# turboderp-org/exllamav2

Hardware: NVIDIA H100
Metric: decode tokens/sec (bs=1) Llama2-7B EXL2-4.0bpw (higher is better)
Workload: dtype fp16 (int2-8 weights, fp32 accumulate)

## Files before the change

exllamav2_b200/csrc/common.cuh:

```cuda
#pragma once
#include <cuda_fp16.h>
#include <cuda_runtime.h>
#include <stdint.h>
#include <stdio.h>
#include <stdlib.h>
#include <string.h>

#include <atomic>

#include "../../include/exl2_b200.h"
#include "layout.h"

namespace exl2b {

void set_error(const char* fmt, ...);
extern std::atomic<uint64_t> g_launch_count;

#define EXL2B_CUDA(call)                                                                              \
    do {                                                                                              \
        cudaError_t _e = (call);                                                                      \
        if (_e != cudaSuccess) {                                                                      \
            exl2b::set_error("%s failed: %s (%s:%d)", #call, cudaGetErrorString(_e), __FILE__, __LINE__); \
            return -1;                                                                                \
        }                                                                                             \
// ... 83 lines not shown
        : "memory");
}
__device__ __forceinline__ void bulk_copy_g2s(uint32_t dst_smem, const void* src, uint32_t bytes, uint32_t bar) {
    asm volatile("cp.async.bulk.shared::cluster.global.mbarrier::complete_tx::bytes [%0], [%1], %2, [%3];" ::"r"(dst_smem),
                 "l"(src), "r"(bytes), "r"(bar)
                 : "memory");
}

__device__ __forceinline__ void bulk_prefetch_l2(const void* src, uint32_t bytes) {
    asm volatile("cp.async.bulk.prefetch.L2.global [%0], %1;" ::"l"(src), "r"(bytes) : "memory");
}

__device__ __forceinline__ void mma16816(float (&d)[4], const uint32_t* a, uint32_t b0, uint32_t b1) {
    asm("mma.sync.aligned.m16n8k16.row.col.f32.f16.f16.f32 {%0,%1,%2,%3}, {%4,%5,%6,%7}, {%8,%9}, {%0,%1,%2,%3};"
        : "+f"(d[0]), "+f"(d[1]), "+f"(d[2]), "+f"(d[3])
        : "r"(a[0]), "r"(a[1]), "r"(a[2]), "r"(a[3]), "r"(b0), "r"(b1));
}

__device__ __forceinline__ uint4 lds128(uint32_t addr) {
    uint4 v;
    asm volatile("ld.shared.v4.u32 {%0,%1,%2,%3}, [%4];" : "=r"(v.x), "=r"(v.y), "=r"(v.z), "=r"(v.w) : "r"(addr));
    return v;
}
__device__ __forceinline__ uint2 lds64(uint32_t addr) {
    uint2 v;
    asm volatile("ld.shared.v2.u32 {%0,%1}, [%2];" : "=r"(v.x), "=r"(v.y) : "r"(addr));
    return v;
}
__device__ __forceinline__ uint32_t lds32(uint32_t addr) {
    uint32_t v;
    asm volatile("ld.shared.u32 %0, [%1];" : "=r"(v) : "r"(addr));
    return v;
}
#endif

}
```

exllamav2_b200/csrc/gemv_i8.cu:

```cuda
#include <string.h>

#include <algorithm>
#include <map>
#include <mutex>
#include <string>
#include <vector>

#include "gemv_i8.cuh"

namespace exl2b {

constexpr int I8_MAX_WARPS = 16;
constexpr int I8_MAX_CTAS = 320;

struct I8Mat {
    const uint8_t* packed;
    const void* wtab;
    const half* bias;
    half* c;
    half* c_perm;
    const uint16_t* out_invperm;
    int N, blk_base, clear;
};

constexpr uint32_t DF_FLUSH = 1, DF_BLOCK_DONE = 2, DF_GPTQ = 4;
constexpr int I8_BARS = 8;

struct I8Params {
    I8Mat mat[I8_MAX_MATS];
    const uint4* plan_desc;
    const uint32_t* plan_first;
    const uint32_t* plan_cta;
    const uint32_t* plan_red;
    int num_mats, K, KS;
    const uint16_t* perm;
    const half* x;
    const half* x2;
    const half* norm_w;
    float norm_eps;
    int mode, x_permuted;
    int norm_permuted;
    int l1_hints;
    int l2_prefetch;
    int arena;
    int busy_ctas;
    unsigned int* slot_cnt;
    unsigned long long* dbg;
    int dbg_cta;
    unsigned long long* dbg_rec;
};

struct I8Smem {
    uint32_t act, asum, ascale, emit, total;
};
__host__ __device__ inline I8Smem i8_smem_map(int warps, int arena, int KS) {
    auto up = [](uint32_t x) { return (x + 15u) & ~15u; };
    I8Smem m;
    m.act = up((uint32_t)warps * (uint32_t)arena);
    m.asum = up(m.act + (uint32_t)KS * 64u);
    m.ascale = up(m.asum + (uint32_t)KS * 4u);
    m.emit = up(m.ascale + (uint32_t)(KS / 4 + 1) * 4u);
    m.total = up(m.emit + (uint32_t)warps * 256u);
    return m;
}

__device__ __forceinline__ int dp4a_us(uint32_t a, uint32_t b, int c) {
    int d;
    asm("dp4a.u32.s32 %0, %1, %2, %3;" : "=r"(d) : "r"(a), "r"(b), "r"(c));
    return d;
}
__device__ __forceinline__ int dp4a_uu(uint32_t a, uint32_t b, int c) {
    int d;
    asm("dp4a.u32.u32 %0, %1, %2, %3;" : "=r"(d) : "r"(a), "r"(b), "r"(c));
    return d;
}

__device__ __forceinline__ uint4 ldg_keep(const uint4* p) {
    uint4 v;
    asm volatile("ld.global.nc.L1::evict_last.v4.u32 {%0,%1,%2,%3}, [%4];" : "=r"(v.x), "=r"(v.y), "=r"(v.z), "=r"(v.w) : "l"(p));
    return v;
}
__device__ __forceinline__ uint32_t ldg_pass_u16(const void* p) {
    unsigned short v;
    asm volatile("ld.global.nc.L1::no_allocate.u16 %0, [%1];" : "=h"(v) : "l"(p));
    return v;
}
__device__ __forceinline__ uint32_t ldg_pass_u32(const void* p) {
    uint32_t v;
    asm volatile("ld.global.nc.L1::no_allocate.u32 %0, [%1];" : "=r"(v) : "l"(p));
    return v;
}

template <int BITS>
__device__ __forceinline__ void consume_slab(uint32_t wb, uint32_t xs, int lane, int (&am)[4], int (&ae)[2]) {
    constexpr int Pm = plane_main(BITS), Pe = plane_extra(BITS);
    if constexpr (BITS == 4) {
        const uint4 w4 = lds128(wb + lane * 16);
#pragma unroll
        for (int hf = 0; hf < 2; ++hf) {
            const uint4 xh = lds128(xs + hf * 16), xl = lds128(xs + 32 + hf * 16);
            const uint32_t wa = hf ? w4.z : w4.x, wc = hf ? w4.w : w4.y;
            const uint32_t lo0 = wa & 0x0f0f0f0fu, hi0 = wa & 0xf0f0f0f0u, lo1 = wc & 0x0f0f0f0fu, hi1 = wc & 0xf0f0f0f0u;
            am[0] = dp4a_us(lo0, xh.x, am[0]);
            am[1] = dp4a_uu(lo0, xl.x, am[1]);
            am[2] = dp4a_us(hi0, xh.y, am[2]);
            am[3] = dp4a_uu(hi0, xl.y, am[3]);
            am[0] = dp4a_us(lo1, xh.z, am[0]);
            am[1] = dp4a_uu(lo1, xl.z, am[1]);
            am[2] = dp4a_us(hi1, xh.w, am[2]);
            am[3] = dp4a_uu(hi1, xl.w, am[3]);
        }
        return;
    }
    uint32_t XH[8], XL[8];
    {
        const uint4 h0 = lds128(xs), h1 = lds128(xs + 16), l0 = lds128(xs + 32), l1 = lds128(xs + 48);
        XH[0] = h0.x; XH[1] = h0.y; XH[2] = h0.z; XH[3] = h0.w; XH[4] = h1.x; XH[5] = h1.y; XH[6] = h1.z; XH[7] = h1.w;
        XL[0] = l0.x; XL[1] = l0.y; XL[2] = l0.z; XL[3] = l0.w; XL[4] = l1.x; XL[5] = l1.y; XL[6] = l1.z; XL[7] = l1.w;
    }
    if constexpr (Pm == 4) {
        const uint4 w4 = lds128(wb + lane * 16);
        const uint32_t W[4] = {w4.x, w4.y, w4.z, w4.w};
#pragma unroll
// ... 144 lines not shown
#define I8_STAMP(i) do { if (P.dbg) { if (blockIdx.x == P.dbg_cta && tid == 0) P.dbg[i] = i8_gtimer(); if ((i) == 0 && tid == 0) atomicMin(P.dbg + 6, i8_gtimer()); } } while (0)

template <int I8_WARPS>
__global__ void __launch_bounds__(I8_WARPS * 32, 2) gemv_i8_kernel(const __grid_constant__ I8Params P) {
    constexpr int I8_THREADS = I8_WARPS * 32;
    extern __shared__ __align__(128) uint8_t smem[];
    __shared__ uint64_t bars[I8_WARPS * I8_BARS];
    __shared__ float s_red[I8_WARPS];

    const int tid = threadIdx.x, warp = tid >> 5, lane = tid & 31;
    const int KS = P.KS;
    I8_STAMP(0);
    if (P.dbg_rec && tid == 0 && blockIdx.x < 160) P.dbg_rec[blockIdx.x * 4] = i8_gtimer();
    if (tid < I8_WARPS * I8_BARS) mbar_init(smem_addr(&bars[tid]), 1);
    mbar_fence_init();
    __syncthreads();
    griddep_launch_dependents();

    if ((int)blockIdx.x >= P.busy_ctas) {
        if (tid == 0) {
            while (*reinterpret_cast<volatile unsigned int*>(P.slot_cnt) < (unsigned)P.busy_ctas) __nanosleep(200);
            if (atomicAdd(P.slot_cnt, 1u) == gridDim.x - 1u) *reinterpret_cast<volatile unsigned int*>(P.slot_cnt) = 0u;
        }
        return;
    }

    const uint32_t cinfo = __ldg(P.plan_cta + blockIdx.x);
    const int blk0 = (int)(cinfo & 0xffffu), nb = (int)(cinfo >> 16);
    const uint32_t fw0 = __ldg(P.plan_first + blockIdx.x * I8_WARPS + warp), fw1 = __ldg(P.plan_first + blockIdx.x * I8_WARPS + warp + 1);
    const uint32_t f0 = fw0 & 0x3ffffffu, f1 = fw1 & 0x3ffffffu;
    const int nst = (int)(f1 - f0), n_pre = (int)(fw0 >> 26);
    const uint4* const list = P.plan_desc + f0;

    const I8Smem sm = i8_smem_map(I8_WARPS, P.arena, KS);
    uint8_t* const act_g = smem + sm.act;
    int* const asum_s = reinterpret_cast<int*>(smem + sm.asum);
    float* const ascale_s = reinterpret_cast<float*>(smem + sm.ascale);
    float* const emit_base = reinterpret_cast<float*>(smem + sm.emit);
    uint32_t sbase;
    asm volatile("mov.u32 %0, %1;" : "=r"(sbase) : "r"(smem_addr(smem)));
    const uint32_t ring = sbase + (uint32_t)warp * (uint32_t)P.arena;
    const uint32_t act = sbase + sm.act, asum = sbase + sm.asum, ascale = sbase + sm.ascale;
    uint32_t bar0;
    asm volatile("mov.u32 %0, %1;" : "=r"(bar0) : "r"(smem_addr(&bars[warp * I8_BARS])));

    uint32_t mi_cur = 0u;
    const uint8_t* pk_cur = P.mat[0].packed;
    const uint8_t* wt_cur = reinterpret_cast<const uint8_t*>(P.mat[0].wtab);
    auto select_mat = [&](uint32_t mi) {
        if (mi != mi_cur) {
            mi_cur = mi;
            pk_cur = mi == 0 ? P.mat[0].packed : (mi == 1 ? P.mat[1].packed : P.mat[2].packed);
            wt_cur = reinterpret_cast<const uint8_t*>(mi == 0 ? P.mat[0].wtab : (mi == 1 ? P.mat[1].wtab : P.mat[2].wtab));
        }
    };
    auto issue_stages = [&](int s0, int cnt, uint4 d) {
        if (lane < cnt) {
            const int s = s0 + lane;
            const uint32_t mi = (d.z >> 22) & 3u;
            const uint8_t* pk = mi == 0 ? P.mat[0].packed : (mi == 1 ? P.mat[1].packed : P.mat[2].packed);
            const uint32_t bytes = ((d.z >> 24) & 0xffu) << 7;
            const uint32_t bar = bar0 + ((uint32_t)s & (I8_BARS - 1)) * 8u;
            mbar_arrive_expect_tx(bar, bytes);
            bulk_copy_g2s(ring + ((d.w >> 16) & 0xffu) * 128u, pk + d.x, bytes, bar);
        }
    };
    auto load_req = [&](int s0) -> uint4 {
        uint4 d = make_uint4(0u, 0u, 0u, 0u);
        if (lane < I8_BARS && s0 + lane < nst) d = P.l1_hints ? ldg_keep(list + s0 + lane) : __ldg(list + s0 + lane);
        return d;
    };
    auto fetch_scale = [&](uint4 d) -> uint32_t {
        select_mat((d.z >> 22) & 3u);
        const uint32_t idx = d.y + (uint32_t)lane;
        if (P.l1_hints)
            return (d.z & (DF_GPTQ << 18)) ? ldg_pass_u32(reinterpret_cast<const uint32_t*>(wt_cur) + idx)
                                            : ldg_pass_u16(reinterpret_cast<const unsigned short*>(wt_cur) + idx);
        return (d.z & (DF_GPTQ << 18)) ? __ldg(reinterpret_cast<const uint32_t*>(wt_cur) + idx)
                                        : (uint32_t)__ldg(reinterpret_cast<const unsigned short*>(wt_cur) + idx);
    };
    uint4 dcur = make_uint4(0u, 0u, 0u, 0u);
    if (nst > 0) dcur = P.l1_hints ? ldg_keep(list) : __ldg(list);
    I8_STAMP(8);
    issue_stages(0, n_pre, load_req(0));
    int next_req = n_pre;
    if (P.l2_prefetch)
        for (int s0 = n_pre; s0 < nst; s0 += 32) {
            const int s = s0 + lane;
            if (s < nst) {
                const uint4 d = __ldg(list + s);
                const uint32_t mi = (d.z >> 22) & 3u;
                const uint8_t* pk = mi == 0 ? P.mat[0].packed : (mi == 1 ? P.mat[1].packed : P.mat[2].packed);
                bulk_prefetch_l2(pk + d.x, ((d.z >> 24) & 0xffu) << 7);
            }
        }
    uint32_t wraw = 0u;
    if (nst > 0) wraw = fetch_scale(dcur);
    I8_STAMP(9);

    const int n_oct = P.K >> 3;
    const bool gather_x = P.perm != nullptr && !P.x_permuted;
    constexpr int PF = 3;
    uint4 pv[PF], wv[PF];
#pragma unroll
    for (int r = 0; r < PF; ++r) {
        const int o = r * I8_THREADS + tid;
        pv[r] = make_uint4(0, 0, 0, 0);
        wv[r] = make_uint4(0, 0, 0, 0);
        if (o < n_oct) {
            if (P.perm && (gather_x || !P.norm_permuted)) pv[r] = __ldg(reinterpret_cast<const uint4*>(P.perm + o * 8));
            if (P.mode == I8_RMSNORM) {
                if (P.perm && !P.norm_permuted) {
                    const uint16_t* pi = reinterpret_cast<const uint16_t*>(&pv[r]);
                    uint16_t* wo = reinterpret_cast<uint16_t*>(&wv[r]);
#pragma unroll
                    for (int e = 0; e < 8; ++e) wo[e] = __half_as_ushort(__ldg(P.norm_w + pi[e]));
                } else {
                    wv[r] = __ldg(reinterpret_cast<const uint4*>(P.norm_w + o * 8));
                }
            }
        }
    }

    I8_STAMP(1);
    griddep_wait();
    I8_STAMP(2);
    if (P.dbg_rec && tid == 0 && blockIdx.x < 160) P.dbg_rec[blockIdx.x * 4 + 1] = i8_gtimer();

    float sumsq = 0.f;
    const bool two_in = (P.mode == I8_SILU_MUL || P.mode == I8_GELU_MUL);
// ... 110 lines not shown
                    wreg = __ldg(reinterpret_cast<const uint4*>(P.norm_w + o * 8));
                }
            }
        }
        stage_round(o, pidx, wreg, false, make_uint4(0, 0, 0, 0));
    }
    if (P.mode == I8_RMSNORM) {
#pragma unroll
        for (int s = 16; s > 0; s >>= 1) sumsq += __shfl_xor_sync(0xffffffffu, sumsq, s);
        if (lane == 0) s_red[warp] = sumsq;
    }
    __syncthreads();
    I8_STAMP(3);
    float rrms = 1.f;
    if (P.mode == I8_RMSNORM) {
        float t = 0.f;
#pragma unroll
        for (int i = 0; i < I8_WARPS; ++i) t += s_red[i];
        rrms = rsqrtf(t * (1.0f / (float)P.K) + P.norm_eps);
    }

    uint32_t red0 = 0u;
    I8OutPre opre0 = {0u, 0u};
    if (warp < nb) {
        red0 = __ldg(P.plan_red + blk0 + warp);
        if (red0 & 0xffffu) opre0 = out_pre(P, blk0 + warp, lane);
    }

    int am[4] = {0, 0, 0, 0}, ae[2] = {0, 0};
    float tot = 0.f;
    int S = 0, blk_slabs = 0, emits = 0;
#pragma unroll 1
    for (int s = 0; s < nst; ++s) {
        const uint4 d = dcur;
        if (s + 1 < nst) dcur = P.l1_hints ? ldg_keep(list + s + 1) : __ldg(list + s + 1);
        const int nreq = (int)((d.w >> 24) & 15u);
        const uint4 dreq = load_req(next_req);
        mbar_wait(bar0 + ((uint32_t)s & (I8_BARS - 1)) * 8u, ((uint32_t)s >> 3) & 1u);
        const int ks = (int)(d.z & 0x7ffu), n = (int)((d.z >> 11) & 7u), bits = (int)((d.z >> 14) & 15u);
        const uint32_t slot = ring + ((d.w >> 16) & 0xffu) * 128u;
        const uint32_t xs = act + (uint32_t)ks * 64u, as = asum + (uint32_t)ks * 4u;
        {
            int bsel = bits;
            auto opaque = [&]() { asm volatile("" : "+r"(bsel)); return bsel; };
            if (bsel == 4) S += consume_stage<4>(slot, n, xs, as, lane, am, ae);
            else if (opaque() == 5) S += consume_stage<5>(slot, n, xs, as, lane, am, ae);
            else if (opaque() == 6) S += consume_stage<6>(slot, n, xs, as, lane, am, ae);
            else if (opaque() == 3) S += consume_stage<3>(slot, n, xs, as, lane, am, ae);
            else if (opaque() == 8) S += consume_stage<8>(slot, n, xs, as, lane, am, ae);
            else S += consume_stage<2>(slot, n, xs, as, lane, am, ae);
        }
        __syncwarp();
        {
            issue_stages(next_req, nreq, dreq);
            next_req += nreq;
        }
        blk_slabs += n;
        if (d.z & (DF_FLUSH << 18)) {
            int v = ((am[0] << 8) + am[1]) + (((am[2] << 8) + am[3]) >> 4) + (((ae[0] << 8) + ae[1]) << plane_main(bits));
            const float ws = __half2float(__ushort_as_half((unsigned short)(wraw & 0xffffu)));
            const int zero = (d.z & (DF_GPTQ << 18)) ? (int)(wraw >> 16) : (1 << (bits - 1));
            v -= zero * S;
            tot = fmaf((float)v, ws * __uint_as_float(lds32(ascale + (uint32_t)(ks >> 2) * 4u)), tot);
            am[0] = am[1] = am[2] = am[3] = 0;
            ae[0] = ae[1] = 0;
            S = 0;
            if (s + 1 < nst) wraw = fetch_scale(dcur);
            if (d.z & (DF_BLOCK_DONE << 18)) {
                const int blk = blk0 + (int)(d.w & 0xffffu);
                if (blk_slabs == KS) {
                    finalize_block(P, blk, lane, out_pre(P, blk, lane), tot * rrms);
                } else {
                    if (emits >= 2) __trap();
                    emit_base[(warp * 2 + emits) * 32 + lane] = tot;
                    ++emits;
                }
                tot = 0.f;
                blk_slabs = 0;
            }
        }
    }
    I8_STAMP(4);
    __syncthreads();
    I8_STAMP(5);

    for (int b = warp; b < nb; b += I8_WARPS) {
        const uint32_t rd = (b == warp) ? red0 : __ldg(P.plan_red + blk0 + b);
        uint32_t m = rd & 0xffffu;
        if (m == 0u) continue;
        int w = __ffs(m) - 1;
        float v = emit_base[(w * 2 + (int)((rd >> 16) & 1u)) * 32 + lane];
        for (m &= m - 1u; m; m &= m - 1u) {
            w = __ffs(m) - 1;
            v += emit_base[(w * 2) * 32 + lane];
        }
        finalize_block(P, blk0 + b, lane, (b == warp) ? opre0 : out_pre(P, blk0 + b, lane), v * rrms);
    }
    if (tid == 0 && atomicAdd(P.slot_cnt, 1u) == gridDim.x - 1u) *reinterpret_cast<volatile unsigned int*>(P.slot_cnt) = 0u;
    if (P.dbg && lane == 0) atomicMax(P.dbg + 7, i8_gtimer());
    if (P.dbg_rec && tid == 0 && blockIdx.x < 160) {
// ... 57 lines not shown
        if (acc + bytes[b] > lo) { out[++c] = (unsigned short)b; acc = 0; }
        acc += bytes[b];
    }
    out[++c] = (unsigned short)nb;
    *used = c;
}

__global__ void gather_rows_kernel(half* __restrict__ out, const half* __restrict__ w, const uint16_t* __restrict__ perm, int K) {
    const int i = blockIdx.x * blockDim.x + threadIdx.x;
    if (i < K) out[i] = w[perm[i]];
}
static std::mutex g_normp_mutex;
static int i8_permuted_norm(QMatrix* q, const half* norm_w, cudaStream_t stream, const half** out) {
    std::lock_guard<std::mutex> lk(g_normp_mutex);
    if (q->normp_src != norm_w) {
        cudaStreamCaptureStatus cs = cudaStreamCaptureStatusNone;
        cudaStreamIsCapturing(stream, &cs);
        if (cs != cudaStreamCaptureStatusNone) { *out = nullptr; return 0; }
        if (!q->normp_buf) EXL2B_CUDA(cudaMalloc(&q->normp_buf, (size_t)q->v.K * sizeof(half)));
        gather_rows_kernel<<<(q->v.K + 255) / 256, 256, 0, stream>>>(q->normp_buf, norm_w, q->v.perm, q->v.K);
        g_launch_count++;
        EXL2B_CUDA(cudaGetLastError());
        q->normp_src = norm_w;
    }
    *out = q->normp_buf;
    return 0;
}

struct I8Plan {
    uint4* d_desc = nullptr;
    uint32_t* d_first = nullptr;
    uint32_t* d_cta = nullptr;
    uint32_t* d_red = nullptr;
    int ctas = 0, lcap = 0, arena = 0;
};
struct I8PlanMat {
    int N, KS, is_gptq, num_regions;
    uint32_t blk_stream_bytes;
    QRegion reg[MAX_REGIONS];
};
static std::map<std::string, I8Plan> g_plans[64];
static std::mutex g_plan_mutex;

static void i8_build_lists(const I8PlanMat* mats, int nm, const unsigned short* cta_blk, int C, int warps, int arena,
                           std::vector<uint4>& desc, std::vector<uint32_t>& first, std::vector<uint32_t>& cta, std::vector<uint32_t>& red,
                           int* lcap) {
    const int KS = mats[0].KS;
    int blk_base[I8_MAX_MATS + 1] = {0};
    for (int i = 0; i < nm; ++i) blk_base[i + 1] = blk_base[i] + (mats[i].N + 31) / 32;
    *lcap = 1;
    red.assign(blk_base[nm], 0u);
    for (int c = 0; c < C; ++c) {
        const int blk0 = cta_blk[c], nb = (int)cta_blk[c + 1] - blk0;
        cta.push_back((uint32_t)blk0 | ((uint32_t)nb << 16));
        const long long units = (long long)nb * KS;
        for (int w = 0; w < warps; ++w) {
            first.push_back((uint32_t)desc.size());
            const int l0 = (int)((units * w) / warps), l1 = (int)((units * (w + 1)) / warps);
            int lin = l0;
            while (lin < l1) {
                const int b = lin / KS, ks = lin - b * KS, blk = blk0 + b;
                int mi = 0;
                while (mi + 1 < nm && blk >= blk_base[mi + 1]) ++mi;
                const I8PlanMat& m = mats[mi];
                int r = 0;
                while (r + 1 < m.num_regions && ks >= m.reg[r + 1].ks_begin) ++r;
                const QRegion& rg = m.reg[r];
// ... 38 lines not shown
                struct Live { int idx; uint32_t off, size; };
                std::vector<Live> live;
                uint32_t off = 0;
                int last_dep = -1;
                for (size_t s = 0; s < nst; ++s) {
                    const uint4& d = desc[w0 + s];
                    const uint32_t size = ((d.z >> 11) & 7u) * ((d.z >> 14) & 15u) * 128u;
                    if (off + size > (uint32_t)arena) off = 0;
                    auto overlaps = [&](const Live& l) { return l.off < off + size && off < l.off + l.size; };
                    for (;;) {
                        bool hit = false;
                        for (const Live& l : live) hit = hit || overlaps(l);
                        if (!hit && (int)live.size() < I8_BARS) break;
                        last_dep = live.front().idx;
                        live.erase(live.begin());
                    }
                    dep[s] = last_dep;
                    live.push_back(Live{(int)s, off, size});
                    desc[w0 + s].w |= (off / 128u) << 16;
                    off += size;
                }
            }
            int n_pre = 0;
            for (size_t s = 0; s < nst; ++s) {
                if (dep[s] < 0) ++n_pre;
                else desc[w0 + dep[s]].w += 1u << 24;
            }
            first.back() |= (uint32_t)n_pre << 26;
        }
    }
    first.push_back((uint32_t)desc.size());
}

static int i8_get_plan(int device, const I8PlanMat* mats, int nm, int sms, int warps, I8Plan* out) {
    std::string key((const char*)mats, sizeof(I8PlanMat) * nm);
    const int extra[3] = {nm, sms, warps};
    key.append((const char*)extra, sizeof(extra));
    std::lock_guard<std::mutex> lk(g_plan_mutex);
    auto it = g_plans[device].find(key);
    if (it != g_plans[device].end()) { *out = it->second; return 0; }

    I8Plan pl;
    std::vector<uint32_t> blk_bytes;
    for (int i = 0; i < nm; ++i) {
        for (int b = 0; b < (mats[i].N + 31) / 32; ++b) blk_bytes.push_back(mats[i].blk_stream_bytes);
    }
    EXL2B_REQUIRE(blk_bytes.size() < 65535, "too many column blocks (%zu)", blk_bytes.size());
    EXL2B_REQUIRE((long long)blk_bytes.size() * mats[0].KS < (1ll << 30), "problem too large for 32-bit unit arithmetic");
    unsigned short cta_blk[I8_MAX_CTAS + 1];
    i8_partition_blocks(blk_bytes, sms, cta_blk, &pl.ctas);
    static const int smem_budget = [] { const char* e = getenv("EXL2B_I8_SMEM"); return e ? atoi(e) : 111 * 1024; }();
    std::vector<uint4> desc;
    std::vector<uint32_t> first, cta, red;
    pl.arena = 8192;
    for (;;) {
        desc.clear(); first.clear(); cta.clear();
        i8_build_lists(mats, nm, cta_blk, pl.ctas, warps, pl.arena, desc, first, cta, red, &pl.lcap);
        if ((int)i8_smem_map(warps, pl.arena, mats[0].KS).total <= smem_budget || pl.arena <= 2048) break;
        pl.arena -= 128;
    }
    EXL2B_REQUIRE(desc.size() < (1u << 26), "too many stages");
    EXL2B_CUDA(cudaMalloc(&pl.d_desc, desc.size() * sizeof(uint4) + 16));
    EXL2B_CUDA(cudaMalloc(&pl.d_first, first.size() * 4));
    EXL2B_CUDA(cudaMalloc(&pl.d_cta, cta.size() * 4));
    EXL2B_CUDA(cudaMemcpy(pl.d_desc, desc.data(), desc.size() * sizeof(uint4), cudaMemcpyHostToDevice));
    EXL2B_CUDA(cudaMemcpy(pl.d_first, first.data(), first.size() * 4, cudaMemcpyHostToDevice));
    EXL2B_CUDA(cudaMemcpy(pl.d_cta, cta.data(), cta.size() * 4, cudaMemcpyHostToDevice));
    EXL2B_CUDA(cudaMalloc(&pl.d_red, red.size() * 4 + 4));
    EXL2B_CUDA(cudaMemcpy(pl.d_red, red.data(), red.size() * 4, cudaMemcpyHostToDevice));
    g_plans[device][key] = pl;
    *out = pl;
    return 0;
}

int gemv_i8_launch(int device, cudaStream_t stream, const I8Out* outs, int nm, const I8Input& in) {
    EXL2B_REQUIRE(nm >= 1 && nm <= I8_MAX_MATS, "bad matrix count %d", nm);
    EXL2B_REQUIRE(device >= 0 && device < 64, "bad device %d", device);
    EXL2B_REQUIRE(in.x, "null input row");
    EXL2B_REQUIRE(in.mode != I8_RMSNORM || in.norm_w, "RMSNorm prologue without a weight");
    EXL2B_REQUIRE((in.mode != I8_SILU_MUL && in.mode != I8_GELU_MUL) || in.x2, "act*mul prologue without the second operand");
    static const int warps = [] {
        const char* e = getenv("EXL2B_I8_WARPS");
        const int w = e ? atoi(e) : 16;
        return (w == 12 || w == 8) ? w : 16;
    }();
    static bool attr_set[64] = {false};
    if (!attr_set[device]) {
        EXL2B_CUDA(cudaFuncSetAttribute(gemv_i8_kernel<16>, cudaFuncAttributeMaxDynamicSharedMemorySize, 200 * 1024));
        EXL2B_CUDA(cudaFuncSetAttribute(gemv_i8_kernel<12>, cudaFuncAttributeMaxDynamicSharedMemorySize, 200 * 1024));
        EXL2B_CUDA(cudaFuncSetAttribute(gemv_i8_kernel<8>, cudaFuncAttributeMaxDynamicSharedMemorySize, 200 * 1024));
        attr_set[device] = true;
    }

    I8Params P = {};
    P.num_mats = nm;
    P.K = outs[0].q->v.K;
    P.KS = outs[0].q->v.KS;
    P.perm = outs[0].q->v.perm;
    P.x = in.x;
    P.x2 = in.x2;
    P.norm_w = in.norm_w;
    P.norm_eps = in.norm_eps;
    P.mode = in.mode;
    P.x_permuted = in.x_permuted;
    if (in.mode == I8_RMSNORM && P.perm) {
        const half* wp = nullptr;
        int rcn = i8_permuted_norm(const_cast<QMatrix*>(outs[0].q), in.norm_w, stream, &wp);
        if (rcn) return rcn;
        if (wp) { P.norm_w = wp; P.norm_permuted = 1; }
    }
    I8PlanMat pm[I8_MAX_MATS];
    memset(pm, 0, sizeof(pm));
    int blk = 0;
    for (int i = 0; i < nm; ++i) {
        const QMatrix* q = outs[i].q;
        EXL2B_REQUIRE(q && outs[i].c, "null matrix / output");
        const QMatView& v = q->v;
        EXL2B_REQUIRE(v.layout == LAYOUT_TC, "matrix is not in the default (LAYOUT_TC) layout");
        EXL2B_REQUIRE(v.KS == P.KS, "fused matrices must share K");
        EXL2B_REQUIRE((v.perm == nullptr) == (P.perm == nullptr), "fused matrices must share their row permutation");
        EXL2B_REQUIRE(q->wtab, "matrix has no scale table");
        EXL2B_REQUIRE(q->packed_bytes < (1ull << 32), "matrix too large for 32-bit stage offsets");
        I8Mat& m = P.mat[i];
        m.packed = reinterpret_cast<const uint8_t*>(v.packed);
        m.wtab = q->wtab;
        m.bias = v.bias;
        m.c = outs[i].c;
        m.c_perm = outs[i].c_perm;
        m.out_invperm = outs[i].out_invperm;
        m.clear = outs[i].clear;
        m.N = v.N;
        m.blk_base = blk;
        blk += (v.N + 31) / 32;
        pm[i].N = v.N;
        pm[i].KS = v.KS;
        pm[i].is_gptq = v.is_gptq;
        pm[i].num_regions = v.num_regions;
        pm[i].blk_stream_bytes = v.blk_stream_bytes;
        for (int r = 0; r < v.num_regions; ++r) pm[i].reg[r] = v.reg[r];
    }
    EXL2B_REQUIRE(P.KS <= 2048, "K = %d exceeds the stage descriptor (K <= 65536)", P.K);
    I8Plan pl;
    static const int double_mb = [] { const char* e = getenv("EXL2B_I8_DOUBLE_MB"); return e ? atoi(e) : 0; }();
    unsigned long long launch_bytes = 0;
    for (int i = 0; i < nm; ++i) launch_bytes += outs[i].q->packed_bytes;
    const int slots = (double_mb > 0 && launch_bytes >= (unsigned long long)double_mb << 20) ? 2 : 1;
    const int grid_ctas = std::min(device_sm_count(device) * slots, I8_MAX_CTAS);
    int rc = i8_get_plan(device, pm, nm, grid_ctas, warps, &pl);
    if (rc) return rc;
    P.plan_desc = pl.d_desc;
    P.plan_first = pl.d_first;
    P.plan_cta = pl.d_cta;
    P.plan_red = pl.d_red;
    P.arena = pl.arena;
    P.busy_ctas = pl.ctas;
    static const int l2pf = [] { const char* e = getenv("EXL2B_I8_L2PF"); return e ? atoi(e) : 0; }();
    P.l2_prefetch = l2pf;
    static const int l1h = [] { const char* e = getenv("EXL2B_I8_L1HINT"); return e ? atoi(e) : 0; }();
    P.l1_hints = l1h;
    const size_t smem_total = i8_smem_map(warps, P.arena, P.KS).total;
    EXL2B_REQUIRE(smem_total <= 200 * 1024, "shared memory budget exceeded (%zu bytes, K = %d)", smem_total, P.K);
    extern unsigned long long* g_dbg;
    extern int g_dbg_cta, g_dbg_slot;
    P.dbg = g_dbg ? g_dbg + 32 * (g_dbg_slot++ % 64) : nullptr;
    P.dbg_cta = g_dbg_cta;
    extern unsigned long long* g_dbg_rec;
    P.dbg_rec = (g_dbg_rec && P.dbg) ? g_dbg_rec + (size_t)((g_dbg_slot - 1) % 64) * 160 * 4 : nullptr;
    static unsigned int* slot_cnts[64] = {nullptr};
    static std::atomic<unsigned> launch_seq{0};
    if (!slot_cnts[device]) {
        EXL2B_CUDA(cudaMalloc(&slot_cnts[device], 128 * sizeof(unsigned int)));
        EXL2B_CUDA(cudaMemset(slot_cnts[device], 0, 128 * sizeof(unsigned int)));
    }
    P.slot_cnt = slot_cnts[device] + (launch_seq.fetch_add(1) % 127u);
    const int C = slot_holders_disabled() ? pl.ctas : std::max(pl.ctas, grid_ctas);
    if (warps == 16) EXL2B_CUDA(launch_pdl_f("i8", gemv_i8_kernel<16>, dim3(C), dim3(16 * 32), smem_total, stream, P));
    else if (warps == 12) EXL2B_CUDA(launch_pdl_f("i8", gemv_i8_kernel<12>, dim3(C), dim3(12 * 32), smem_total, stream, P));
    else EXL2B_CUDA(launch_pdl_f("i8", gemv_i8_kernel<8>, dim3(C), dim3(8 * 32), smem_total, stream, P));
    return 0;
}

}

extern "C" int exl2b_debug_partition(const uint32_t* block_bytes, int num_blocks, int ctas, uint16_t* out, int* used) {
    EXL2B_REQUIRE(block_bytes && out && used && num_blocks > 0 && ctas > 0 && ctas <= exl2b::I8_MAX_CTAS, "bad argument");
    std::vector<uint32_t> b(block_bytes, block_bytes + num_blocks);
    exl2b::i8_partition_blocks(b, ctas, out, used);
    return 0;
}

extern "C" int exl2b_debug_plan(int N, int KS, int is_gptq, uint32_t blk_stream_bytes, const int* regions, int num_regions, int ctas, int warps,
                                int slot_bytes, uint32_t* desc, int cap_desc, uint32_t* first, int* ctas_used, int* n_desc, int* lcap,
                                uint32_t* red) {
    EXL2B_REQUIRE(regions && desc && first && ctas_used && n_desc && lcap, "null argument");
    EXL2B_REQUIRE(num_regions >= 1 && num_regions <= exl2b::MAX_REGIONS && ctas > 0 && ctas <= exl2b::I8_MAX_CTAS && warps > 0, "bad argument");
    exl2b::I8PlanMat m;
    memset(&m, 0, sizeof(m));
    m.N = N; m.KS = KS; m.is_gptq = is_gptq; m.num_regions = num_regions; m.blk_stream_bytes = blk_stream_bytes;
    for (int r = 0; r < num_regions; ++r)
        m.reg[r] = exl2b::QRegion{regions[5 * r], regions[5 * r + 1], regions[5 * r + 2], regions[5 * r + 3], (uint32_t)regions[5 * r + 4]};
    std::vector<uint32_t> bb((N + 31) / 32, blk_stream_bytes);
    unsigned short cta_blk[exl2b::I8_MAX_CTAS + 1];
    exl2b::i8_partition_blocks(bb, ctas, cta_blk, ctas_used);
    std::vector<uint4> d;
    std::vector<uint32_t> f, c, r;
    exl2b::i8_build_lists(&m, 1, cta_blk, *ctas_used, warps, slot_bytes, d, f, c, r, lcap);
    EXL2B_REQUIRE((int)d.size() <= cap_desc, "descriptor buffer too small (%zu)", d.size());
    memcpy(desc, d.data(), d.size() * sizeof(uint4));
    memcpy(first, f.data(), f.size() * 4);
    if (red) memcpy(red, r.data(), r.size() * 4);
    *n_desc = (int)d.size();
    return 0;
}
```

include/exl2_b200.h:

```cpp
#ifndef EXL2_B200_H
#define EXL2_B200_H

#include <stddef.h>
#include <stdint.h>

#ifdef __cplusplus
extern "C" {
#endif

typedef void* exl2b_stream_t;
typedef void* exl2b_qmatrix_t;
typedef void* exl2b_qattn_t;
typedef void* exl2b_qmlp_t;

const char* exl2b_last_error(void);
int exl2b_version(void);
uint64_t exl2b_launch_count(void);

typedef struct exl2b_qmatrix_desc {
    int device;
    int height;
    int width;
    int groups;
    uint32_t* q_weight;
// ... 48 lines not shown
    int hidden_size, num_heads, num_kv_heads, head_dim;
    int has_residual;
    int rope_style;
    int sincos_size;
} exl2b_qattn_desc;
int exl2b_qattn_create(const exl2b_qattn_desc* desc, exl2b_qattn_t* out);
int exl2b_qattn_destroy(exl2b_qattn_t h);
int exl2b_qattn_forward_1(exl2b_qattn_t h, const uint16_t* x, int batch, int q_len, int past_len, const int32_t* past_lens,
                          uint16_t* q, uint16_t* k, uint16_t* v, const uint16_t* sin, const uint16_t* cos, exl2b_stream_t stream);
int exl2b_qattn_forward_2(exl2b_qattn_t h, uint16_t* x, const uint16_t* attn_out, int batch, int q_len, exl2b_stream_t stream);

typedef struct exl2b_qmlp_desc {
    const uint16_t* layernorm;
    float norm_epsilon;
    exl2b_qmatrix_t gate, up, down;
    int hidden_size, intermediate_size;
    int act_gelu;
    int has_residual;
} exl2b_qmlp_desc;
int exl2b_qmlp_create(const exl2b_qmlp_desc* desc, exl2b_qmlp_t* out);
int exl2b_qmlp_destroy(exl2b_qmlp_t h);
int exl2b_qmlp_forward(exl2b_qmlp_t h, uint16_t* x, int rows, uint16_t* temp_a, uint16_t* temp_b, exl2b_stream_t stream);
int exl2b_qmlp_forward_gateup(exl2b_qmlp_t h, const uint16_t* x, int rows, uint16_t* temp_a, exl2b_stream_t stream);

int exl2b_gemm_half_q_half_host(exl2b_qmatrix_t h, const uint16_t* a_host, uint16_t* c_host, int m, exl2b_stream_t stream);

int exl2b_debug_set(int ctas_per_sm, unsigned long long* stamps, int cta);

int exl2b_debug_partition(const uint32_t* block_bytes, int num_blocks, int ctas, uint16_t* out, int* used);
int exl2b_debug_set_records(unsigned long long* records);
int exl2b_debug_plan(int N, int KS, int is_gptq, uint32_t blk_stream_bytes, const int* regions, int num_regions, int ctas, int warps,
                     int slot_bytes, uint32_t* desc, int cap_desc, uint32_t* first, int* ctas_used, int* n_desc, int* lcap,
                     uint32_t* red);

int exl2b_paged_attn_decode(const uint16_t* q, const uint16_t* k_new, const uint16_t* v_new, uint16_t* k_cache,
                            uint16_t* v_cache, const int32_t* cache_seqlens, const int32_t* block_table, uint16_t* out,
                            int batch, int q_len, int num_heads, int num_kv_heads, int head_dim, int page_size,
                            int pages_per_seq, float softmax_scale, exl2b_stream_t stream);

int exl2b_paged_attn_decode_q4(const uint16_t* q, const uint16_t* k_new, const uint16_t* v_new, uint8_t* k_cache,
                               uint16_t* k_scales, uint8_t* v_cache, uint16_t* v_scales, const int32_t* cache_seqlens,
                               const int32_t* block_table, uint16_t* out, int batch, int q_len, int num_heads,
                               int num_kv_heads, int head_dim, int page_size, int pages_per_seq, float softmax_scale,
                               exl2b_qmatrix_t out_consumer, exl2b_stream_t stream);

int exl2b_paged_attn_decode_q4_ex(const uint16_t* q, const uint16_t* k_new, const uint16_t* v_new, uint8_t* k_cache,
                                  uint16_t* k_scales, uint8_t* v_cache, uint16_t* v_scales, const int32_t* cache_seqlens,
                                  const int32_t* block_table, uint16_t* out, int batch, int q_len, int num_heads,
                                  int num_kv_heads, int head_dim, int page_size, int pages_per_seq, float softmax_scale,
                                  exl2b_qmatrix_t out_consumer, const uint16_t* rope_sin, const uint16_t* rope_cos,
                                  int rope_style, int sincos_size, exl2b_stream_t stream);
int exl2b_paged_attn_decode_q(const uint16_t* q, const uint16_t* k_new, const uint16_t* v_new, uint8_t* k_cache,
                              uint16_t* k_scales, uint8_t* v_cache, uint16_t* v_scales, const int32_t* cache_seqlens,
                              const int32_t* block_table, uint16_t* out, int batch, int q_len, int num_heads,
                              int num_kv_heads, int head_dim, int page_size, int pages_per_seq, float softmax_scale,
                              exl2b_qmatrix_t out_consumer, const uint16_t* rope_sin, const uint16_t* rope_cos,
                              int rope_style, int sincos_size, int wbits, exl2b_stream_t stream);
int exl2b_paged_attn_status(int device, int* status);
int exl2b_paged_attn_clear_status(int device);

typedef struct {
    exl2b_qmatrix_t consumers[3];
    int num_consumers;
    const uint16_t* norm_weight;
} exl2b_chain_t;
int exl2b_qattn_forward_1_ex(exl2b_qattn_t h, const uint16_t* x, int batch, int q_len, int past_len, const int32_t* past_lens,
// ... 15 lines not shown
```

Baseline: 416.9.

## Stage stage descriptors and scale rows into shared memory via TMA bulk copies

The int8 GEMV warp loop no longer reads stage descriptors and per-column scale rows from global memory with per-lane __ldg. Instead they travel alongside the weight slab in the same mbarrier-tracked bulk copies, into a per-warp descriptor window and scale ring in shared memory. This takes dependent global-load latency off the critical path of each stage, and it drops the L1-hint env knob. In exchange it uses more shared memory, which can shrink the weight arena, and it adds a small 16-byte bulk copy per stage.

```diff
diff --git a/exllamav2_b200/csrc/common.cuh b/exllamav2_b200/csrc/common.cuh
--- a/exllamav2_b200/csrc/common.cuh
+++ b/exllamav2_b200/csrc/common.cuh
@@ -139,6 +139,15 @@
     asm volatile("ld.shared.u32 %0, [%1];" : "=r"(v) : "r"(addr));
     return v;
 }
+__device__ __forceinline__ uint32_t lds_u16(uint32_t addr) {
+    unsigned short v;
+    asm volatile("ld.shared.u16 %0, [%1];" : "=h"(v) : "r"(addr));
+    return v;
+}
+__device__ __forceinline__ void stu128(uint32_t addr, uint4 v) {
+    asm volatile("st.shared.v4.u32 [%0], {%1,%2,%3,%4};" ::"r"(addr), "r"(v.x), "r"(v.y), "r"(v.z), "r"(v.w) : "memory");
+}
+__device__ __forceinline__ void fence_proxy_async() { asm volatile("fence.proxy.async.shared::cta;" ::: "memory"); }
 #endif
 
 }
diff --git a/exllamav2_b200/csrc/gemv_i8.cu b/exllamav2_b200/csrc/gemv_i8.cu
--- a/exllamav2_b200/csrc/gemv_i8.cu
+++ b/exllamav2_b200/csrc/gemv_i8.cu
@@ -25,6 +25,7 @@
 
 constexpr uint32_t DF_FLUSH = 1, DF_BLOCK_DONE = 2, DF_GPTQ = 4;
 constexpr int I8_BARS = 8;
+constexpr int I8_LWIN = 2 * I8_BARS;
 
 struct I8Params {
     I8Mat mat[I8_MAX_MATS];
@@ -40,9 +41,9 @@
     float norm_eps;
     int mode, x_permuted;
     int norm_permuted;
-    int l1_hints;
     int l2_prefetch;
     int arena;
+    int srow;
     int busy_ctas;
     unsigned int* slot_cnt;
     unsigned long long* dbg;
@@ -51,16 +52,18 @@
 };
 
 struct I8Smem {
-    uint32_t act, asum, ascale, emit, total;
+    uint32_t act, asum, ascale, emit, scl, lst, total;
 };
-__host__ __device__ inline I8Smem i8_smem_map(int warps, int arena, int KS) {
+__host__ __device__ inline I8Smem i8_smem_map(int warps, int arena, int KS, int srow) {
     auto up = [](uint32_t x) { return (x + 15u) & ~15u; };
     I8Smem m;
     m.act = up((uint32_t)warps * (uint32_t)arena);
     m.asum = up(m.act + (uint32_t)KS * 64u);
     m.ascale = up(m.asum + (uint32_t)KS * 4u);
     m.emit = up(m.ascale + (uint32_t)(KS / 4 + 1) * 4u);
-    m.total = up(m.emit + (uint32_t)warps * 256u);
+    m.scl = up(m.emit + (uint32_t)warps * 256u);
+    m.lst = up(m.scl + (uint32_t)(warps * I8_BARS * srow));
+    m.total = up(m.lst + (uint32_t)(warps * I8_LWIN * 16));
     return m;
 }
 
@@ -73,22 +76,6 @@
     int d;
     asm("dp4a.u32.u32 %0, %1, %2, %3;" : "=r"(d) : "r"(a), "r"(b), "r"(c));
     return d;
-}
-
-__device__ __forceinline__ uint4 ldg_keep(const uint4* p) {
-    uint4 v;
-    asm volatile("ld.global.nc.L1::evict_last.v4.u32 {%0,%1,%2,%3}, [%4];" : "=r"(v.x), "=r"(v.y), "=r"(v.z), "=r"(v.w) : "l"(p));
-    return v;
-}
-__device__ __forceinline__ uint32_t ldg_pass_u16(const void* p) {
-    unsigned short v;
-    asm volatile("ld.global.nc.L1::no_allocate.u16 %0, [%1];" : "=h"(v) : "l"(p));
-    return v;
-}
-__device__ __forceinline__ uint32_t ldg_pass_u32(const void* p) {
-    uint32_t v;
-    asm volatile("ld.global.nc.L1::no_allocate.u32 %0, [%1];" : "=r"(v) : "l"(p));
-    return v;
 }
 
 template <int BITS>
@@ -299,7 +286,7 @@
     const int nst = (int)(f1 - f0), n_pre = (int)(fw0 >> 26);
     const uint4* const list = P.plan_desc + f0;
 
-    const I8Smem sm = i8_smem_map(I8_WARPS, P.arena, KS);
+    const I8Smem sm = i8_smem_map(I8_WARPS, P.arena, KS, P.srow);
     uint8_t* const act_g = smem + sm.act;
     int* const asum_s = reinterpret_cast<int*>(smem + sm.asum);
     float* const ascale_s = reinterpret_cast<float*>(smem + sm.ascale);
@@ -308,48 +295,37 @@
     asm volatile("mov.u32 %0, %1;" : "=r"(sbase) : "r"(smem_addr(smem)));
     const uint32_t ring = sbase + (uint32_t)warp * (uint32_t)P.arena;
     const uint32_t act = sbase + sm.act, asum = sbase + sm.asum, ascale = sbase + sm.ascale;
+    const uint32_t sring = sbase + sm.scl + (uint32_t)(warp * I8_BARS * P.srow), lwin = sbase + sm.lst + (uint32_t)(warp * I8_LWIN * 16);
     uint32_t bar0;
     asm volatile("mov.u32 %0, %1;" : "=r"(bar0) : "r"(smem_addr(&bars[warp * I8_BARS])));
 
-    uint32_t mi_cur = 0u;
-    const uint8_t* pk_cur = P.mat[0].packed;
-    const uint8_t* wt_cur = reinterpret_cast<const uint8_t*>(P.mat[0].wtab);
-    auto select_mat = [&](uint32_t mi) {
-        if (mi != mi_cur) {
-            mi_cur = mi;
-            pk_cur = mi == 0 ? P.mat[0].packed : (mi == 1 ? P.mat[1].packed : P.mat[2].packed);
-            wt_cur = reinterpret_cast<const uint8_t*>(mi == 0 ? P.mat[0].wtab : (mi == 1 ? P.mat[1].wtab : P.mat[2].wtab));
-        }
-    };
     auto issue_stages = [&](int s0, int cnt, uint4 d) {
         if (lane < cnt) {
             const int s = s0 + lane;
             const uint32_t mi = (d.z >> 22) & 3u;
             const uint8_t* pk = mi == 0 ? P.mat[0].packed : (mi == 1 ? P.mat[1].packed : P.mat[2].packed);
+            const uint8_t* wt = reinterpret_cast<const uint8_t*>(mi == 0 ? P.mat[0].wtab : (mi == 1 ? P.mat[1].wtab : P.mat[2].wtab));
             const uint32_t bytes = ((d.z >> 24) & 0xffu) << 7;
-            const uint32_t bar = bar0 + ((uint32_t)s & (I8_BARS - 1)) * 8u;
-            mbar_arrive_expect_tx(bar, bytes);
+            const uint32_t esz = (d.z & (DF_GPTQ << 18)) ? 4u : 2u;
+            const uint32_t sbytes = (d.z & (DF_FLUSH << 18)) ? 32u * esz : 0u;
+            const bool lnext = s + I8_BARS < nst;
+            const uint32_t slot = (uint32_t)s & (I8_BARS - 1);
+            const uint32_t bar = bar0 + slot * 8u;
+            mbar_arrive_expect_tx(bar, bytes + sbytes + (lnext ? 16u : 0u));
             bulk_copy_g2s(ring + ((d.w >> 16) & 0xffu) * 128u, pk + d.x, bytes, bar);
+            if (sbytes) bulk_copy_g2s(sring + slot * (uint32_t)P.srow, wt + (size_t)d.y * esz, sbytes, bar);
+            if (lnext) bulk_copy_g2s(lwin + ((uint32_t)(s + I8_BARS) & (I8_LWIN - 1)) * 16u, list + s + I8_BARS, 16u, bar);
         }
     };
-    auto load_req = [&](int s0) -> uint4 {
-        uint4 d = make_uint4(0u, 0u, 0u, 0u);
-        if (lane < I8_BARS && s0 + lane < nst) d = P.l1_hints ? ldg_keep(list + s0 + lane) : __ldg(list + s0 + lane);
-        return d;
-    };
-    auto fetch_scale = [&](uint4 d) -> uint32_t {
-        select_mat((d.z >> 22) & 3u);
-        const uint32_t idx = d.y + (uint32_t)lane;
-        if (P.l1_hints)
-            return (d.z & (DF_GPTQ << 18)) ? ldg_pass_u32(reinterpret_cast<const uint32_t*>(wt_cur) + idx)
-                                            : ldg_pass_u16(reinterpret_cast<const unsigned short*>(wt_cur) + idx);
-        return (d.z & (DF_GPTQ << 18)) ? __ldg(reinterpret_cast<const uint32_t*>(wt_cur) + idx)
-                                        : (uint32_t)__ldg(reinterpret_cast<const unsigned short*>(wt_cur) + idx);
-    };
-    uint4 dcur = make_uint4(0u, 0u, 0u, 0u);
-    if (nst > 0) dcur = P.l1_hints ? ldg_keep(list) : __ldg(list);
+    uint4 dfirst = make_uint4(0u, 0u, 0u, 0u);
+    if (lane < I8_BARS && lane < nst) {
+        dfirst = __ldg(list + lane);
+        stu128(lwin + (uint32_t)lane * 16u, dfirst);
+    }
+    fence_proxy_async();
+    __syncwarp();
     I8_STAMP(8);
-    issue_stages(0, n_pre, load_req(0));
+    issue_stages(0, n_pre, dfirst);
     int next_req = n_pre;
     if (P.l2_prefetch)
         for (int s0 = n_pre; s0 < nst; s0 += 32) {
@@ -361,8 +337,6 @@
                 bulk_prefetch_l2(pk + d.x, ((d.z >> 24) & 0xffu) << 7);
             }
         }
-    uint32_t wraw = 0u;
-    if (nst > 0) wraw = fetch_scale(dcur);
     I8_STAMP(9);
 
     const int n_oct = P.K >> 3;
@@ -539,11 +513,10 @@
     int S = 0, blk_slabs = 0, emits = 0;
 #pragma unroll 1
     for (int s = 0; s < nst; ++s) {
-        const uint4 d = dcur;
-        if (s + 1 < nst) dcur = P.l1_hints ? ldg_keep(list + s + 1) : __ldg(list + s + 1);
+        const uint4 d = lds128(lwin + ((uint32_t)s & (I8_LWIN - 1)) * 16u);
         const int nreq = (int)((d.w >> 24) & 15u);
-        const uint4 dreq = load_req(next_req);
-        mbar_wait(bar0 + ((uint32_t)s & (I8_BARS - 1)) * 8u, ((uint32_t)s >> 3) & 1u);
+        const uint32_t slot8 = (uint32_t)s & (I8_BARS - 1);
+        mbar_wait(bar0 + slot8 * 8u, ((uint32_t)s >> 3) & 1u);
         const int ks = (int)(d.z & 0x7ffu), n = (int)((d.z >> 11) & 7u), bits = (int)((d.z >> 14) & 15u);
         const uint32_t slot = ring + ((d.w >> 16) & 0xffu) * 128u;
         const uint32_t xs = act + (uint32_t)ks * 64u, as = asum + (uint32_t)ks * 4u;
@@ -557,6 +530,12 @@
             else if (opaque() == 8) S += consume_stage<8>(slot, n, xs, as, lane, am, ae);
             else S += consume_stage<2>(slot, n, xs, as, lane, am, ae);
         }
+        uint4 dreq = make_uint4(0u, 0u, 0u, 0u);
+        if (lane < nreq) dreq = lds128(lwin + ((uint32_t)(next_req + lane) & (I8_LWIN - 1)) * 16u);
+        uint32_t wraw = 0u;
+        if (d.z & (DF_FLUSH << 18))
+            wraw = (d.z & (DF_GPTQ << 18)) ? lds32(sring + slot8 * (uint32_t)P.srow + (uint32_t)lane * 4u)
+                                           : lds_u16(sring + slot8 * (uint32_t)P.srow + (uint32_t)lane * 2u);
         __syncwarp();
         {
             issue_stages(next_req, nreq, dreq);
@@ -572,7 +551,6 @@
             am[0] = am[1] = am[2] = am[3] = 0;
             ae[0] = ae[1] = 0;
             S = 0;
-            if (s + 1 < nst) wraw = fetch_scale(dcur);
             if (d.z & (DF_BLOCK_DONE << 18)) {
                 const int blk = blk0 + (int)(d.w & 0xffffu);
                 if (blk_slabs == KS) {
@@ -696,7 +674,7 @@
     uint32_t* d_first = nullptr;
     uint32_t* d_cta = nullptr;
     uint32_t* d_red = nullptr;
-    int ctas = 0, lcap = 0, arena = 0;
+    int ctas = 0, lcap = 0, arena = 0, srow = 64;
 };
 struct I8PlanMat {
     int N, KS, is_gptq, num_regions;
@@ -801,6 +779,31 @@
     first.push_back((uint32_t)desc.size());
 }
 
+static int i8_plan_host(const I8PlanMat* mats, int nm, int sms, int warps, I8Plan& pl, std::vector<uint4>& desc,
+                        std::vector<uint32_t>& first, std::vector<uint32_t>& cta, std::vector<uint32_t>& red) {
+    std::vector<uint32_t> blk_bytes;
+    for (int i = 0; i < nm; ++i) {
+        for (int b = 0; b < (mats[i].N + 31) / 32; ++b) blk_bytes.push_back(mats[i].blk_stream_bytes);
+    }
+    EXL2B_REQUIRE(blk_bytes.size() < 65535, "too many column blocks (%zu)", blk_bytes.size());
+    EXL2B_REQUIRE((long long)blk_bytes.size() * mats[0].KS < (1ll << 30), "problem too large for 32-bit unit arithmetic");
+    unsigned short cta_blk[I8_MAX_CTAS + 1];
+    i8_partition_blocks(blk_bytes, sms, cta_blk, &pl.ctas);
+    static const int smem_budget = [] { const char* e = getenv("EXL2B_I8_SMEM"); return e ? atoi(e) : 111 * 1024; }();
+    pl.srow = 64;
+    for (int i = 0; i < nm; ++i)
+        if (mats[i].is_gptq) pl.srow = 128;
+    pl.arena = 8192;
+    for (;;) {
+        desc.clear(); first.clear(); cta.clear();
+        i8_build_lists(mats, nm, cta_blk, pl.ctas, warps, pl.arena, desc, first, cta, red, &pl.lcap);
+        if ((int)i8_smem_map(warps, pl.arena, mats[0].KS, pl.srow).total <= smem_budget || pl.arena <= 2048) break;
+        pl.arena -= 128;
+    }
+    EXL2B_REQUIRE(desc.size() < (1u << 26), "too many stages");
+    return 0;
+}
+
 static int i8_get_plan(int device, const I8PlanMat* mats, int nm, int sms, int warps, I8Plan* out) {
     std::string key((const char*)mats, sizeof(I8PlanMat) * nm);
     const int extra[3] = {nm, sms, warps};
@@ -810,25 +813,10 @@
     if (it != g_plans[device].end()) { *out = it->second; return 0; }
 
     I8Plan pl;
-    std::vector<uint32_t> blk_bytes;
-    for (int i = 0; i < nm; ++i) {
-        for (int b = 0; b < (mats[i].N + 31) / 32; ++b) blk_bytes.push_back(mats[i].blk_stream_bytes);
-    }
-    EXL2B_REQUIRE(blk_bytes.size() < 65535, "too many column blocks (%zu)", blk_bytes.size());
-    EXL2B_REQUIRE((long long)blk_bytes.size() * mats[0].KS < (1ll << 30), "problem too large for 32-bit unit arithmetic");
-    unsigned short cta_blk[I8_MAX_CTAS + 1];
-    i8_partition_blocks(blk_bytes, sms, cta_blk, &pl.ctas);
-    static const int smem_budget = [] { const char* e = getenv("EXL2B_I8_SMEM"); return e ? atoi(e) : 111 * 1024; }();
     std::vector<uint4> desc;
     std::vector<uint32_t> first, cta, red;
-    pl.arena = 8192;
-    for (;;) {
-        desc.clear(); first.clear(); cta.clear();
-        i8_build_lists(mats, nm, cta_blk, pl.ctas, warps, pl.arena, desc, first, cta, red, &pl.lcap);
-        if ((int)i8_smem_map(warps, pl.arena, mats[0].KS).total <= smem_budget || pl.arena <= 2048) break;
-        pl.arena -= 128;
-    }
-    EXL2B_REQUIRE(desc.size() < (1u << 26), "too many stages");
+    const int rc = i8_plan_host(mats, nm, sms, warps, pl, desc, first, cta, red);
+    if (rc) return rc;
     EXL2B_CUDA(cudaMalloc(&pl.d_desc, desc.size() * sizeof(uint4) + 16));
     EXL2B_CUDA(cudaMalloc(&pl.d_first, first.size() * 4));
     EXL2B_CUDA(cudaMalloc(&pl.d_cta, cta.size() * 4));
@@ -889,6 +877,7 @@
         EXL2B_REQUIRE(v.KS == P.KS, "fused matrices must share K");
         EXL2B_REQUIRE((v.perm == nullptr) == (P.perm == nullptr), "fused matrices must share their row permutation");
         EXL2B_REQUIRE(q->wtab, "matrix has no scale table");
+        EXL2B_REQUIRE(v.N % 8 == 0, "width %d is not a multiple of 8", v.N);
         EXL2B_REQUIRE(q->packed_bytes < (1ull << 32), "matrix too large for 32-bit stage offsets");
         I8Mat& m = P.mat[i];
         m.packed = reinterpret_cast<const uint8_t*>(v.packed);
@@ -922,12 +911,11 @@
     P.plan_cta = pl.d_cta;
     P.plan_red = pl.d_red;
     P.arena = pl.arena;
+    P.srow = pl.srow;
     P.busy_ctas = pl.ctas;
     static const int l2pf = [] { const char* e = getenv("EXL2B_I8_L2PF"); return e ? atoi(e) : 0; }();
     P.l2_prefetch = l2pf;
-    static const int l1h = [] { const char* e = getenv("EXL2B_I8_L1HINT"); return e ? atoi(e) : 0; }();
-    P.l1_hints = l1h;
-    const size_t smem_total = i8_smem_map(warps, P.arena, P.KS).total;
+    const size_t smem_total = i8_smem_map(warps, P.arena, P.KS, P.srow).total;
     EXL2B_REQUIRE(smem_total <= 200 * 1024, "shared memory budget exceeded (%zu bytes, K = %d)", smem_total, P.K);
     extern unsigned long long* g_dbg;
     extern int g_dbg_cta, g_dbg_slot;
@@ -981,3 +969,35 @@
     *n_desc = (int)d.size();
     return 0;
 }
+
+extern "C" int exl2b_debug_i8_plan(const int* mats, int nm, int ctas, int warps, uint32_t* desc, int cap_desc, uint32_t* first,
+                                   int cap_first, int* info) {
+    EXL2B_REQUIRE(mats && desc && first && info, "null argument");
+    EXL2B_REQUIRE(nm >= 1 && nm <= exl2b::I8_MAX_MATS && ctas > 0 && ctas <= exl2b::I8_MAX_CTAS && warps > 0, "bad argument");
+    exl2b::I8PlanMat pm[exl2b::I8_MAX_MATS];
+    memset(pm, 0, sizeof(pm));
+    for (int i = 0; i < nm; ++i) {
+        const int* r = mats + i * (5 + 5 * exl2b::MAX_REGIONS);
+        EXL2B_REQUIRE(r[4] >= 1 && r[4] <= exl2b::MAX_REGIONS && r[1] == mats[1], "bad matrix %d", i);
+        pm[i].N = r[0]; pm[i].KS = r[1]; pm[i].is_gptq = r[2]; pm[i].blk_stream_bytes = (uint32_t)r[3]; pm[i].num_regions = r[4];
+        for (int g = 0; g < r[4]; ++g) {
+            const int* q = r + 5 + 5 * g;
+            pm[i].reg[g] = exl2b::QRegion{q[0], q[1], q[2], q[3], (uint32_t)q[4]};
+        }
+    }
+    exl2b::I8Plan pl;
+    std::vector<uint4> d;
+    std::vector<uint32_t> f, c, red;
+    const int rc = exl2b::i8_plan_host(pm, nm, ctas, warps, pl, d, f, c, red);
+    if (rc) return rc;
+    EXL2B_REQUIRE((int)d.size() <= cap_desc && (int)f.size() <= cap_first, "output buffers too small (%zu, %zu)", d.size(), f.size());
+    memcpy(desc, d.data(), d.size() * sizeof(uint4));
+    memcpy(first, f.data(), f.size() * 4);
+    info[0] = pl.ctas;
+    info[1] = (int)d.size();
+    info[2] = pl.arena;
+    info[3] = pl.srow;
+    info[4] = (int)exl2b::i8_smem_map(warps, pl.arena, pm[0].KS, pl.srow).total;
+    info[5] = pl.lcap;
+    return 0;
+}
diff --git a/include/exl2_b200.h b/include/exl2_b200.h
--- a/include/exl2_b200.h
+++ b/include/exl2_b200.h
@@ -104,6 +104,8 @@
 int exl2b_debug_plan(int N, int KS, int is_gptq, uint32_t blk_stream_bytes, const int* regions, int num_regions, int ctas, int warps,
                      int slot_bytes, uint32_t* desc, int cap_desc, uint32_t* first, int* ctas_used, int* n_desc, int* lcap,
                      uint32_t* red);
+int exl2b_debug_i8_plan(const int* mats, int nm, int ctas, int warps, uint32_t* desc, int cap_desc, uint32_t* first, int cap_first,
+                        int* info);
 
 int exl2b_paged_attn_decode(const uint16_t* q, const uint16_t* k_new, const uint16_t* v_new, uint16_t* k_cache,
                             uint16_t* v_cache, const int32_t* cache_seqlens, const int32_t* block_table, uint16_t* out,
```

Result: faster. 484.3 (median of 6 runs) (+16.2%).
